# GJ0407790/cuda_ray_tracer

Measured on AMD Instinct MI355X. Metric: Mrays/sec, tenthousand.txt 1080p@16spp, higher is better.
Workload: dtype f32

## Files before the change

### cuda_ray_tracer_amd/api.py

```python
import contextlib
import ctypes as C
import os

from .binding import (LIB_PATH, EXPORTS, MIRT_ERR_ARG, MIRT_RENDER_COUNTERS, MIRT_HIT_NONE, MIRT_HIT_SPHERE, MIRT_HIT_TRIANGLE,
                      MIRT_HIT_PLANE, MIRT_QUERY_ANY_HIT, MIRT_DENOISE_SIGMA_C, MIRT_DENOISE_SIGMA_N, MIRT_DENOISE_SIGMA_P, MirtError, Vec3, Ray,
                      Hit, Camera, Shading, SceneDesc, RenderParams, Stats, MultiStats, TreeNode, lib, _check)

_F32, _U8, _INT, _HIT = ("float32",), ("uint8",), ("int32", "uint32"), ("float32", "int32", "uint32")


def _struct_with(cls, s, fields, what):
    out = cls.from_buffer_copy(bytes(s))
    names = dict(cls._fields_)
    for k, v in fields.items():
        if k not in names:
            raise ValueError(f"{k} is not a {what} field; expected one of {sorted(names)}")
        if names[k] is Vec3 and not isinstance(v, Vec3):
            v = Vec3(*(float(c) for c in v))
        setattr(out, k, v)
    return out


def _camera_with(cam, fields):
    return _struct_with(Camera, cam, fields, "camera")
# ... 79 lines not shown
        self._h = h
        self.build_ms = None

    def stats(self):
        st = Stats()
        _check(lib().mirt_get_stats(self._h, C.byref(st)))
        return st.as_dict()

    def set_option(self, name, value):
        _check(lib().mirt_scene_set_option(self._h, name.encode(), int(value)))

    def get_option(self, name):
        v = C.c_int(0)
        _check(lib().mirt_scene_get_option(self._h, name.encode(), C.byref(v)))
        return v.value

    def camera(self):
        cam = Camera()
        _check(lib().mirt_scene_get_camera(self._h, C.byref(cam)))
        return cam

    def set_camera(self, cam=None, **fields):
        new = _camera_with(cam if cam is not None else self.camera(), fields)
        _check(lib().mirt_scene_set_camera(self._h, C.byref(new)))
        return new

    def lights(self):
        import numpy as np
        from . import layouts
        suns = np.zeros(self.desc.num_suns, dtype=layouts.LIGHT)
# ... 608 lines not shown
```

### cuda_ray_tracer_amd/csrc/api.hip

```cpp
#include "scene_dev.h"
#include "host_scene.h"
#include "material_flags.h"

#include <cmath>
#include <cstdlib>
#include <cstring>
#include <memory>
#include <new>
#include <string>
#include <vector>

using namespace mirt;

namespace {

template <typename T>
int upload(DevBuf<T>& dst, const std::vector<T>& src)
{
  if (src.empty()) return MIRT_OK;
  const int rc = dst.alloc(src.size(), "upload");
  if (rc != MIRT_OK) return rc;
  MIRT_HIP(hipMemcpy(dst, src.data(), sizeof(T) * src.size(), hipMemcpyHostToDevice));
  return MIRT_OK;
}
// ... 48 lines not shown
  for (const OptionDesc& d : OPTIONS)
    if (strcmp(d.name, name) == 0) {
      if (value < d.lo || value > d.hi) { set_error(std::string("mirt_scene_set_option: value out of range for ") + name); return MIRT_ERR_ARG; }
      sc->opt.*(d.field) = value;
      return MIRT_OK;
    }
  set_error(std::string("mirt_scene_set_option: unknown option ") + name);
  return MIRT_ERR_ARG;
}

int mirt_scene_get_option(const MirtScene* sc, const char* name, int* value)
{
  if (!sc || !name || !value) { set_error("mirt_scene_get_option: null argument"); return MIRT_ERR_ARG; }
  for (const OptionDesc& d : OPTIONS)
    if (strcmp(d.name, name) == 0) { *value = sc->opt.*(d.field); return MIRT_OK; }
  set_error(std::string("mirt_scene_get_option: unknown option ") + name);
  return MIRT_ERR_ARG;
}

int mirt_scene_create(const MirtSceneDesc* d, int device, MirtScene** out)
{
  try {
    return scene_create(d, device, out);
  } catch (const std::bad_alloc&) {
    set_error("mirt_scene_create: out of host memory");
    return MIRT_ERR_ARG;
  }
}

}
// ... 78 lines not shown
    sc->wnode_base = wnode_bytes ? (uint32_t)((nodes_bytes + sph_bytes + tri_bytes + 64 + qnode_bytes + 127) / 128 * 128) : 0u;
    sc->nodes = reinterpret_cast<float4*>(sc->heap.get());
  }
  MIRT_TRY(upload(sc->spheres, spheres)); MIRT_TRY(upload(sc->tris, tris));
  MIRT_TRY(upload(sc->tri_verts, verts)); MIRT_TRY(upload(sc->mats, mats));
  MIRT_TRY(upload(sc->refs_in, refs)); MIRT_TRY(upload(sc->planes, planes)); MIRT_TRY(upload(sc->suns, suns)); MIRT_TRY(upload(sc->bulbs, bulbs));
  if (N > 0) {
    const size_t n = (size_t)N;
    MIRT_TRY(sc->codes.alloc(n, "codes")); MIRT_TRY(sc->order.alloc(n, "order"));
    MIRT_TRY(sc->parent.alloc(2 * n - 1, "parent")); MIRT_TRY(sc->boxes.alloc(6 * (2 * n - 1), "boxes"));
    if (N > 1) { MIRT_TRY(sc->child_l.alloc(n - 1, "child_l")); MIRT_TRY(sc->child_r.alloc(n - 1, "child_r")); MIRT_TRY(sc->range.alloc(n - 1, "range")); }
    MIRT_TRY(sc->unit_prim.alloc((size_t)sc->Ns + 3 * (size_t)sc->Nt, "unit_prim"));
    MIRT_TRY(sc->tris_before.alloc(n + 1, "tris_before"));
  }
  MIRT_TRY(sc->bounds_keys.alloc(6, "bounds_keys"));
  MIRT_TRY(sc->qparams.alloc(9, "qparams"));
  MIRT_TRY(sc->tri_boxes.alloc(2 * (size_t)sc->Nt, "tri_boxes"));
  for (RenderCtx& c : sc->ctx) {
    MIRT_TRY(c.counters.alloc(16, "counters"));
    MIRT_HIP(hipMemset(c.counters, 0, 16 * sizeof(unsigned long long)));
  }
  MIRT_TRY(sc->ev0.create()); MIRT_TRY(sc->ev1.create()); MIRT_TRY(sc->so_ev.create());
  for (RenderCtx& c : sc->ctx) {
    MIRT_TRY(c.ev0.create()); MIRT_TRY(c.ev1.create()); MIRT_TRY(c.ev2.create()); MIRT_TRY(c.ev3.create()); MIRT_TRY(c.order_ev.create());
  }
  *out = owner.release();
  return MIRT_OK;
}

}
// ... 315 lines not shown
```

### cuda_ray_tracer_amd/csrc/lbvh_build.hip

```cpp
#include "scene_dev.h"
#include "host_scene.h"

#include <cstdio>
#include <cstring>

namespace mirt {

int hip_fail(hipError_t e, const char* what, const char* file, int line)
{
  char buf[512];
  snprintf(buf, sizeof(buf), "HIP error in %s at line %d: %s (%s)", file, line, hipGetErrorString(e), what);
  set_error(buf);
  return MIRT_ERR_HIP;
}

namespace {

constexpr int BLOCK = 256;

struct Box { float xmin, xmax, ymin, ymax, zmin, zmax; };

MIRT_DEV Box prim_box(uint32_t type, uint32_t id, const float4* __restrict__ spheres, const float4* __restrict__ tri_verts)
{
  Box b;
// ... 406 lines not shown
                                                              uint32_t* __restrict__ unit_prim)
{
  const int j = blockIdx.x * BLOCK + threadIdx.x;
  if (j >= n) return;
  const MirtPrimRef r = refs[order[j]];
  const size_t unit = (size_t)j + 2 * (size_t)tris_before[j];
  if (r.type == 0) {
    prim_region[unit] = spheres[r.id];
    unit_prim[unit] = r.id;
  } else {
    prim_region[unit + 0] = tris[3 * (size_t)r.id + 0];
    prim_region[unit + 1] = tris[3 * (size_t)r.id + 1];
    prim_region[unit + 2] = tris[3 * (size_t)r.id + 2];
    unit_prim[unit + 0] = 0x80000000u | r.id; unit_prim[unit + 1] = 0x80000000u | r.id; unit_prim[unit + 2] = 0x80000000u | r.id;
  }
}

__global__ void __launch_bounds__(BLOCK) refit_pack_kernel(int n, const uint32_t* __restrict__ order, const MirtPrimRef* __restrict__ refs,
                                                           const float4* __restrict__ spheres, const float4* __restrict__ tri_verts,
                                                           const uint32_t* __restrict__ child_l, const uint32_t* __restrict__ child_r,
                                                           const int* __restrict__ parent, uint32_t* __restrict__ arrived,
                                                           float* boxes, float4* __restrict__ nodes, const uint32_t* __restrict__ tris_before,
                                                           const uint2* __restrict__ range, uint32_t prim_base16, float4* __restrict__ tri_boxes)
{
  const int j = blockIdx.x * BLOCK + threadIdx.x;
  if (j >= n) return;
  const uint32_t leaf_base = (uint32_t)(n - 1);
  uint32_t cur = leaf_base + (uint32_t)j;
  const MirtPrimRef r = refs[order[j]];
  const Box b = prim_box(r.type, r.id, spheres, tri_verts);
// ... 44 lines not shown
{
  const int sblocks = (int)((n + SORT_TILE - 1) / SORT_TILE);
  uint32_t *hist = ws, *totals = ws + 256 * (size_t)sblocks;
  hipLaunchKernelGGL(radix_pass_kernel<false>, dim3(sblocks), dim3(BLOCK), 0, stream, keys_in, (const uint32_t*)nullptr, keys_out, vals_out, hist, hist, totals, (int)n, 0, sblocks);
  hipLaunchKernelGGL(row_scan_kernel, dim3(256), dim3(BLOCK), 0, stream, hist, totals, sblocks);
  hipLaunchKernelGGL(radix_pass_kernel<true>, dim3(sblocks), dim3(BLOCK), 0, stream, keys_in, (const uint32_t*)nullptr, keys_out, vals_out, hist, hist, totals, (int)n, 0, sblocks);
  MIRT_HIP(hipGetLastError());
  return MIRT_OK;
}

int build_lbvh(MirtScene* sc, hipStream_t stream)
{
  const int n = sc->N;
  sc->built = false;
  sc->root_ref = REF_NONE;
  if (n == 0) { sc->built = true; sc->build_ms = 0.0f; return MIRT_OK; }

  const int sblocks = (n + SORT_TILE - 1) / SORT_TILE;
  const size_t wwords = 4 * (size_t)n + 256 * (size_t)sblocks + 256 + (size_t)(n > 1 ? n - 1 : 0);
  if (sc->build_ws.cap() < wwords) MIRT_TRY(sc->build_ws.alloc(wwords, "build_ws"));
  MIRT_HIP(hipEventRecord(sc->ev0, stream));
  const int nblk = (n + BLOCK - 1) / BLOCK;
  if (!sc->opt.bounds_as_shipped) {
    static const uint32_t init_keys[6] = {0xffffffffu, 0xffffffffu, 0xffffffffu, 0u, 0u, 0u};
    MIRT_HIP(hipMemcpyAsync(sc->bounds_keys, init_keys, sizeof(init_keys), hipMemcpyHostToDevice, stream));
    const int bgrid = nblk < 512 ? nblk : 512;
    hipLaunchKernelGGL(prim_bounds_kernel, dim3(bgrid), dim3(BLOCK), 0, stream, sc->refs_in, sc->spheres, sc->tri_verts, n, sc->bounds_keys);
  } else {
    static const uint32_t shipped_keys[6] = {0xff800000u, 0xff800000u, 0xff800000u, 0x007fffffu, 0x007fffffu, 0x007fffffu};
    MIRT_HIP(hipMemcpyAsync(sc->bounds_keys, shipped_keys, sizeof(shipped_keys), hipMemcpyHostToDevice, stream));
  }
// ... 7 lines not shown
    const int shift = pass * 8;
    hipLaunchKernelGGL(radix_pass_kernel<false>, dim3(sblocks), dim3(BLOCK), 0, stream, ki, vi, ko, vo, hist, hist, totals, n, shift, sblocks);
    hipLaunchKernelGGL(row_scan_kernel, dim3(256), dim3(BLOCK), 0, stream, hist, totals, sblocks);
    hipLaunchKernelGGL(radix_pass_kernel<true>, dim3(sblocks), dim3(BLOCK), 0, stream, ki, vi, ko, vo, hist, hist, totals, n, shift, sblocks);
    uint32_t* t = ki; ki = ko; ko = t; t = vi; vi = vo; vo = t;
  }
  MIRT_HIP(hipMemcpyAsync(sc->codes, ki, sizeof(uint32_t) * n, hipMemcpyDeviceToDevice, stream));
  MIRT_HIP(hipMemcpyAsync(sc->order, vi, sizeof(uint32_t) * n, hipMemcpyDeviceToDevice, stream));

  uint32_t* arrived = totals + 256;
  if (n > 1) {
    MIRT_HIP(hipMemsetAsync(arrived, 0, sizeof(uint32_t) * (n - 1), stream));
    MIRT_HIP(hipMemsetAsync(sc->parent, 0xff, sizeof(int) * (2 * (size_t)n - 1), stream));
    const int kblk = (n - 1 + BLOCK - 1) / BLOCK;
    hipLaunchKernelGGL(karras_kernel, dim3(kblk), dim3(BLOCK), 0, stream, sc->codes, n, sc->child_l, sc->child_r, sc->parent, sc->range);
  } else {
    MIRT_HIP(hipMemsetAsync(sc->parent, 0xff, sizeof(int), stream));
  }
  const int scan_blocks = (n + SCAN_TILE - 1) / SCAN_TILE;
  uint32_t* const block_sums = k1;
  hipLaunchKernelGGL(tri_scan_kernel<false>, dim3(scan_blocks), dim3(BLOCK), 0, stream, n, sc->order, sc->refs_in, block_sums, sc->tris_before);
  hipLaunchKernelGGL(scan_sums_kernel, dim3(1), dim3(BLOCK), 0, stream, block_sums, scan_blocks);
  hipLaunchKernelGGL(tri_scan_kernel<true>, dim3(scan_blocks), dim3(BLOCK), 0, stream, n, sc->order, sc->refs_in, block_sums, sc->tris_before);
  hipLaunchKernelGGL(scatter_prims_kernel, dim3(nblk), dim3(BLOCK), 0, stream, n, sc->order, sc->refs_in, sc->tris_before, sc->spheres, sc->tris,
                     reinterpret_cast<float4*>(sc->heap + sc->prim_base), sc->unit_prim);
  hipLaunchKernelGGL(refit_pack_kernel, dim3(nblk), dim3(BLOCK), 0, stream, n, sc->order, sc->refs_in, sc->spheres, sc->tri_verts,
                     sc->child_l, sc->child_r, sc->parent, arrived, sc->boxes, sc->nodes, sc->tris_before, sc->range, sc->prim_base / 16u, sc->tri_boxes);
  sc->root_ref_q = REF_NONE;
  if (sc->qnode_base && n > 1 && !sc->opt.bounds_as_shipped) {
    const int kblk = (n - 1 + BLOCK - 1) / BLOCK;
// ... 3 lines not shown
  }
  sc->root_ref_w = REF_NONE;
  if (sc->wnode_base && n > 1 && !sc->opt.bounds_as_shipped) {
    const int kblk = (n - 1 + BLOCK - 1) / BLOCK;
    hipLaunchKernelGGL(pack_wnodes_kernel, dim3(kblk), dim3(BLOCK), 0, stream, n, sc->bounds_keys, sc->child_l, sc->child_r, sc->boxes,
                       sc->order, sc->refs_in, sc->tris_before, sc->range, reinterpret_cast<uint4*>(sc->heap + sc->wnode_base),
                       sc->qparams, sc->wnode_base / 16u, sc->prim_base / 16u);
    sc->root_ref_w = sc->wnode_base / 16u;
  }
  MIRT_HIP(hipGetLastError());
  MIRT_HIP(hipEventRecord(sc->ev1, stream));
  MIRT_HIP(hipStreamSynchronize(stream));
  MIRT_HIP(hipEventElapsedTime(&sc->build_ms, sc->ev0, sc->ev1));
  sc->coord_max = 0.0f;
  sc->grid_ok = false;
  if (n > 1) {
    float rec[12];
    MIRT_HIP(hipMemcpy(rec, sc->nodes, sizeof(rec), hipMemcpyDeviceToHost));
    for (float v : rec) sc->coord_max = fmaxf(sc->coord_max, fabsf(v));
    sc->grid_ok = true;
    for (int k = 0; k < 3; ++k) {
      const float lo = fminf(rec[2 * k], rec[6 + 2 * k]), hi = fmaxf(rec[2 * k + 1], rec[6 + 2 * k + 1]);
      if (!(fmaxf(fabsf(lo), fabsf(hi)) <= 64.0f * (hi - lo))) sc->grid_ok = false;
    }
  }
  sc->root_ref = (n == 1) ? (REF_LEAF | (sc->Nt ? REF_TRI : 0u) | (sc->prim_base / 16u)) : 0u;
  sc->built = true;
  return MIRT_OK;
}

int get_tree(MirtScene* sc, MirtTreeNode* nodes, uint32_t* codes, MirtPrimRef* refs, float* bounds)
// ... 39 lines not shown
```

### cuda_ray_tracer_amd/csrc/render.hip

```cpp
#include "scene_dev.h"
#include "host_scene.h"
#include "shade_common.h"

#include <algorithm>
#include <climits>
#include <cmath>
#include <cstdio>
#include <cstdlib>
#include <cstring>

namespace mirt {
namespace {

constexpr int RBLOCK = 256;
constexpr int MAX_SPP = 4096;
constexpr int MAX_SLAB_ARGS = 4;
#ifndef MIRT_WAVES_PER_SIMD
#define MIRT_WAVES_PER_SIMD 4
#endif
MIRT_DEV bool triangle_leaf_reached(const RenderArgs* __restrict__ ap, uint32_t off16, const f3& o, const f3& d, float t, float tmin, f3& inv)
{
  const RenderArgs* aq = ap;
  asm volatile("" : "+s"(aq));
  const uint32_t id = aq->unit_prim[off16 - aq->prim_base16] & 0x7fffffffu;
  const float4 b0 = aq->tri_boxes[2 * (size_t)id], b1 = aq->tri_boxes[2 * (size_t)id + 1];
  inv = mk3(1.0f / d.x, 1.0f / d.y, 1.0f / d.z);
  const float tx1 = (b0.x - o.x) * inv.x, tx2 = (b0.y - o.x) * inv.x;
  const float ty1 = (b0.z - o.y) * inv.y, ty2 = (b0.w - o.y) * inv.y;
  const float tz1 = (b1.x - o.z) * inv.z, tz2 = (b1.y - o.z) * inv.z;
  const float te = fmaxf(fmaxf(fminf(tx1, tx2), fminf(ty1, ty2)), fminf(tz1, tz2));
  const float tx = fminf(fminf(fmaxf(tx1, tx2), fmaxf(ty1, ty2)), fmaxf(tz1, tz2));
  return te < tx && tx > tmin && te < t;
}

template <bool COUNT, int TABLES, bool QN, int SPECX = 0>
__global__ void __launch_bounds__(TRACE_BLOCK, MIRT_WAVES_PER_SIMD) trace_kernel(const RenderArgs* __restrict__ ap, const HotArgs h)
{
  constexpr int SPEC = SPECX;
  constexpr bool NOTRI = (SPEC & SPEC_NOTRI) != 0;
  constexpr bool WIDE = QN && !NOTRI;
#define MIRT_HELD (QN && !(SPEC & SPEC_NOBULB) && h.reach_check && S.batch_pending && !S.trav && S.li >= h.num_suns && S.li < h.num_suns + h.num_bulbs && \
                   S.refbest != REF_NONE)
  __shared__ __attribute__((aligned(16))) unsigned char lds_raw[STACK_LDS * TRACE_BLOCK * 4];
  __shared__ uint4 lds_rng[2][TRACE_BLOCK];
  __shared__ uint4 lds_park[2][TRACE_BLOCK];
  uint32_t* const lds_stack = reinterpret_cast<uint32_t*>(lds_raw);
  const int tid = threadIdx.x;
  const int lane = tid & 63;
  (void)lane;
  const unsigned char* const heap = reinterpret_cast<const unsigned char*>(h.nodes);
  const uint32_t gid32 = blockIdx.x * (uint32_t)TRACE_BLOCK + (uint32_t)tid;
  const long long gid = (long long)gid32;
  const long long gthreads = (long long)(gridDim.x * (uint32_t)TRACE_BLOCK);
  Counters cn = {0, 0, 0, 0, 0, 0, 0, 0, 0};

// ... 10 lines not shown
  S.pc = 0; S.refr_bounce = 0; S.gi_n = 0; S.state = ST_PRIMARY;
  S.bo = mk3(0, 0, 0); S.rdir = mk3(0, 0, 1); S.li = 0; S.occl = 0ull; S.batch_pending = false; S.has_reflect = false;
  S.o = mk3(0, 0, 0); S.d = mk3(0, 0, 1); S.inv = mk3(0, 0, 1); S.bounce = 0; S.limit = INFINITY; S.shadow = false;
  S.tplane = INFINITY; S.plane_id = -1;
  S.qb = mk3(0, 0, 0); S.qc = mk3(0, 0, 0); S.qsx = S.qsy = S.qsz = 0;
  S.cur = REF_NONE; S.tos = REF_NONE; S.sp = 0; S.tbest = INFINITY; S.refbest = REF_NONE;

  lds_rng[0][tid] = make_uint4(0, 0, 0, 0);
  lds_rng[1][tid] = make_uint4(0, 0, 0, 0);
  lds_park[0][tid] = make_uint4(0, 0, 0, 0);
  lds_park[1][tid] = make_uint4(0, 0, 0, __float_as_uint(1.458f));
  for (;;) {
    const RenderArgs* aq = ap;
    asm volatile("" : "+s"(aq));
    const RenderArgs& a = *aq;
    if (a.reach_check && !S.trav && S.g >= 0 && !(exhausted && S.batch_pending && !MIRT_HELD) && (!S.batch_pending || S.li >= a.num_suns)) {
      if (hit_needs_literal_walk<QN>(a, S)) walk_literally<COUNT, NOTRI>(a, S, cn, gid, gthreads);
    }
    {
      const uint4 r0 = lds_rng[0][tid], r1 = lds_rng[1][tid];
      S.rng.v0 = r0.x; S.rng.v1 = r0.y; S.rng.v2 = r0.z; S.rng.v3 = r0.w;
      S.rng.v4 = r1.x; S.rng.d = r1.y; S.rng.bm_extra = __uint_as_float(r1.z); S.rng.bm_flag = (int)r1.w;
      const uint4 p0 = lds_park[0][tid], p1 = lds_park[1][tid];
      S.L = mk3(__uint_as_float(p0.x), __uint_as_float(p0.y), __uint_as_float(p0.z)); S.alpha = __uint_as_float(p0.w);
      S.wD = mk3(__uint_as_float(p1.x), __uint_as_float(p1.y), __uint_as_float(p1.z)); S.Hior = __uint_as_float(p1.w);
    }
    for (;;) {
      const bool live = !S.trav && S.g >= 0 && !(exhausted && S.batch_pending && !MIRT_HELD);
      if (__ballot(live) == 0) break;
      if (live && S.batch_pending) batch_next<COUNT, QN, RenderArgs, SPEC>(a, S, cn);
// ... 45 lines not shown
      if (exhausted && __ballot(S.g >= 0) == 0) break;
      continue;
    }

    const float tmin = 0.0001f;
    for (;;) {
      const unsigned long long tm = __ballot(S.trav);
      const bool pend = !S.trav && S.batch_pending && !MIRT_HELD;
      const unsigned long long bm = __ballot(pend);
      if (tm == 0 && bm == 0) break;
      const int nwait = __popcll(__ballot(!S.trav && !pend && (S.g >= 0 || !exhausted)));
      const int nlive = __popcll(__ballot(S.g >= 0));
      const bool drain = exhausted && nlive <= h.drain_lanes;
      if (nwait >= h.refill_k || (drain && nwait > 0)) break;
      if (bm != 0 && (__popcll(bm) >= h.batch_k || tm == 0 || drain)) {
        if (pend) batch_next<COUNT, QN, HotArgs, SPEC>(h, S, cn);
      }
      const bool leaf0 = S.trav && (S.cur & REF_LEAF) != 0;
      const unsigned long long lm = __ballot(leaf0);
      const bool do_leaf0 = __popcll(lm) >= h.leaf_k || __ballot(S.trav && !leaf0) == 0 || drain;
      for (int rep = 0; rep < h.reps; ++rep) {
      const bool leaf = S.trav && (S.cur & REF_LEAF) != 0;
      const bool do_leaf = rep == 0 && do_leaf0;
      if (S.trav && (!leaf || do_leaf)) {
        if (COUNT) ++S.steps;
        const float4* rec = reinterpret_cast<const float4*>(heap + (S.cur << 4));
        bool pop = false;
        if (leaf) {
          float t = 0.0f;
          bool hit = false;
          const float4 q0 = rec[0];
          const bool tri = !NOTRI && (S.cur & REF_TRI) != 0;
          if (tri) {
            if (COUNT) cn.tri_tests++;
            const float4 q1 = rec[1], q2 = rec[2];
            hit = triangle_hit(q0, q1, q2, S.o, S.d, t);
// ... 13 lines not shown
              S.tbest = INFINITY; S.refbest = REF_NONE;
            }
          }
          S.tbest = closer ? t : S.tbest;
          S.refbest = closer ? S.cur : S.refbest;
          S.trav = !(closer && S.shadow && t < S.limit);
          pop = S.trav;
        } else {
          if (COUNT) cn.internal_visits++;
          uint32_t noff = S.cur << 4;
          asm volatile("" : "+v"(noff));
          const float4* nrec = reinterpret_cast<const float4*>(heap + noff);
          bool hl, hr;
          float tel, ter;
          uint32_t lref, rref;
#define MIRT_PUSH(v) do { if (S.sp < h.lds_depth) lds_stack[S.sp * TRACE_BLOCK + tid] = S.tos; \
                          else h.stack_spill[(size_t)(S.sp - h.lds_depth) * gthreads + gid] = S.tos; \
                          S.tos = (v); ++S.sp; if (COUNT) cn.max_stack = max(cn.max_stack, (uint32_t)S.sp); } while (0)
          if (WIDE && S.qsx != 0u) {
            const uint4 w0 = *reinterpret_cast<const uint4*>(nrec), w1 = *reinterpret_cast<const uint4*>(nrec + 1);
            const uint4 w2 = *reinterpret_cast<const uint4*>(nrec + 2), w3 = *reinterpret_cast<const uint4*>(nrec + 3);
            const bool h0 = box_q(w0.x, w0.y, w0.z, S.inv, S.qb, S.qc, S.qsx, S.qsy, S.qsz, S.tbest, tmin);
            const bool h1 = box_q(w0.w, w1.x, w1.y, S.inv, S.qb, S.qc, S.qsx, S.qsy, S.qsz, S.tbest, tmin);
            const bool h2 = box_q(w1.z, w1.w, w2.x, S.inv, S.qb, S.qc, S.qsx, S.qsy, S.qsz, S.tbest, tmin);
            const bool h3 = box_q(w2.y, w2.z, w2.w, S.inv, S.qb, S.qc, S.qsx, S.qsy, S.qsz, S.tbest, tmin);
            uint32_t cand = w3.w;
            bool have = h3;
            if (h2 && have) MIRT_PUSH(cand);
            cand = h2 ? w3.z : cand; have = have || h2;
            if (h1 && have) MIRT_PUSH(cand);
            cand = h1 ? w3.y : cand; have = have || h1;
// ... 7 lines not shown
            order_children(hl, hr, tel, ter, NODE_SWAP_ANY | NODE_SWAP_PURE, h.swap_mask, lref, rref);
          } else {
            const float4 q0 = nrec[0], q1 = nrec[1], q2 = nrec[2];
            const uint4 ch = *reinterpret_cast<const uint4*>(nrec + 3);
            box_pair(q0, q1, q2, S.o.x, S.o.y, S.o.z, S.inv.x, S.inv.y, S.inv.z, S.tbest, tmin, hl, hr, tel, ter);
            lref = ch.x; rref = ch.y;
            if (!QN) order_children(hl, hr, tel, ter, ch.z, h.swap_mask, lref, rref);
          }
          const bool both = hl && hr;
          if (both) MIRT_PUSH(rref);
#undef MIRT_PUSH
          S.cur = hl ? lref : (hr ? rref : S.cur);
          pop = !(hl || hr);
        }
        if (pop) {
          S.trav = S.sp != 0;
          S.cur = S.tos;
          S.sp = S.sp > 0 ? S.sp - 1 : 0;
          S.tos = lds_stack[(S.sp < h.lds_depth ? S.sp : 0) * TRACE_BLOCK + tid];
          if (S.sp >= h.lds_depth) S.tos = h.stack_spill[(size_t)(S.sp - h.lds_depth) * gthreads + gid];
        }
      }
      }
    }
  }

  unsigned long long* const counters = COUNT ? ap->counters : nullptr;
  if (COUNT && counters) {
    uint32_t v[9] = {cn.samples, cn.rays, cn.shadow_rays, cn.internal_visits, cn.sphere_tests, cn.tri_tests, cn.mat_fetches, cn.max_stack, cn.traversed};
#pragma unroll
    for (int k = 0; k < 9; ++k) {
      unsigned long long x = v[k];
      if (k == 7) {
#pragma unroll
        for (int off = 32; off > 0; off >>= 1) { unsigned long long y = __shfl_xor(x, off); x = x > y ? x : y; }
// ... 206 lines not shown

struct RenderCall {
  MirtScene* sc; const MirtRenderParams* p;
  void* d_rgba8; void* d_rgba_f32; void* d_accum; const AdaptiveArgs* ax;
  int sample_first, sample_count;
  hipStream_t stream;
  bool sparse() const { return ax && ax->list; }
  bool count() const { return (p->flags & MIRT_RENDER_COUNTERS) != 0; }
};

static int scene_facts(MirtScene* sc, SceneFacts* out)
{
  const int rc = settle_facts(sc);
  if (rc != MIRT_OK) return rc;
  SceneFacts f;
  f.N = sc->N; f.Nt = sc->Nt; f.grid_ok = sc->grid_ok;
  f.has_quantised = sc->root_ref_q != REF_NONE; f.has_wide = sc->root_ref_w != REF_NONE;
  f.colors_finite = sc->colors_finite; f.any_trans = sc->any_trans; f.any_rough = sc->any_rough;
  f.gi = sc->d.gi; f.bounces = sc->d.bounces; f.num_suns = sc->d.num_suns; f.num_bulbs = sc->d.num_bulbs;
  *out = f;
  return MIRT_OK;
}

static int check_call(const RenderCall& c, int64_t* npix)
{
  const char* who = c.ax ? "mirt_render_accumulate_pixels" : (c.d_accum ? "mirt_render_accumulate" : "mirt_render");
  *npix = 0;
  if (!c.sc->built) { set_error(std::string(who) + ": call mirt_build_lbvh first"); return MIRT_ERR_STATE; }
  const int64_t n = local_pixels(c.p);
  if (n < 0 || c.p->spp < 0 || (!c.d_rgba8 && !c.d_accum)) { set_error(std::string(who) + ": bad parameters"); return MIRT_ERR_ARG; }
  if (c.sample_first < 0 || c.sample_count < 1 || (long long)c.sample_first + c.sample_count > MAX_SPP) {
// ... 165 lines not shown

static int sample_table_finish(MirtScene* sc, hipStream_t stream)
{
  MIRT_HIP(hipEventRecord(sc->so_ev, stream));
  sc->so_key = sc->so_pending_key; sc->so_busy = true;
  return MIRT_OK;
}

using TraceKernel = void (*)(const RenderArgs*, HotArgs);
template <bool C, bool Q, int P>
static TraceKernel trace_kernel_tables(bool t8) { return t8 ? trace_kernel<C, 8, Q, P> : trace_kernel<C, 4, Q, P>; }
template <bool C>
static TraceKernel trace_kernel_spec(bool t8, const CallPlan& pl)
{
  const bool both = pl.nobulb && pl.nopend;
  if (pl.qn && pl.notri) return both ? trace_kernel_tables<C, true, SPEC_NOTRI | SPEC_NOBULB | SPEC_NOPEND>(t8) : trace_kernel_tables<C, true, SPEC_NOTRI>(t8);
  if (pl.qn) return both ? trace_kernel_tables<C, true, SPEC_NOBULB | SPEC_NOPEND>(t8) : pl.nobulb ? trace_kernel_tables<C, true, SPEC_NOBULB>(t8) : trace_kernel_tables<C, true, 0>(t8);
  return both ? trace_kernel_tables<C, false, SPEC_NOBULB | SPEC_NOPEND>(t8) : pl.nobulb ? trace_kernel_tables<C, false, SPEC_NOBULB>(t8) : trace_kernel_tables<C, false, 0>(t8);
}
static TraceKernel trace_kernel_for(bool count, bool t8, const CallPlan& pl) { return count ? trace_kernel_spec<true>(t8, pl) : trace_kernel_spec<false>(t8, pl); }

static int launch_slab(const RenderCall& c, RenderCtx& cx, const CallPlan& pl, RenderArgs& a, const HotArgs& h, int slab, long long p0, long long pn,
                       int blocks, TraceKernel kernel)
{
  const hipStream_t stream = c.stream;
  if (c.sc->opt.wavefront != 0) {
    float tms = 0.0f;
    int rc = wavefront_trace(c.sc, cx, a, c.count(), stream, &tms);
    if (rc != MIRT_OK) return rc;
    cx.wf_trace_ms = (cx.wf_trace_ms < 0.0f ? 0.0f : cx.wf_trace_ms) + tms;
// ... 78 lines not shown
    if (measure_chunks) a.chunk_cost = cx.chunk_cost;
  } else if (pl.hand_out == HAND_BY_SAMPLE) {
    rc = sample_table_find(sc, pl, okey, &ordered_samples, &measure_samples);
  }
  if (rc != MIRT_OK) return rc;
  const TraceKernel kernel = trace_kernel_for(count || measure_chunks || measure_samples,
                                              a.needs_rng && a.rng.mode == 0 && a.rng.chunk_bits == 8, pl);

  cx.frame_id = ++sc->frame_seq;
  MIRT_HIP(hipEventRecord(cx.ev0, stream));
  if (measure_chunks) MIRT_HIP(hipMemsetAsync(cx.chunk_cost, 0, 4 * nchunks, stream));
  if (count) { MIRT_HIP(hipMemsetAsync(cx.counters, 0, 8 * sizeof(unsigned long long), stream)); MIRT_HIP(hipMemsetAsync(cx.counters + 11, 0, sizeof(unsigned long long), stream)); }
  cx.wf_trace_ms = -1.0f;
  cx.launches = pl.nslabs;
  cx.node_bytes = pl.node_bytes;
  MIRT_HIP(hipEventRecord(cx.ev1, stream));
  for (int slab = 0; slab < pl.nslabs; ++slab) {
    const long long p0 = (long long)slab * pl.slab_pixels;
    const long long pn = (p0 + pl.slab_pixels < npix ? p0 + pl.slab_pixels : npix) - p0;
    a.pixel_base = p0; a.num_local_pixels = pn; a.num_samples = pn * sample_count;
    a.sample_order = ordered_samples ? sc->so_order + (size_t)p0 * sample_count : nullptr;
    a.sample_key = measure_samples ? sc->so_keys : nullptr;
    if (c.sparse()) {
      a.sample_order = cx.sp_table;
      a.num_samples = (pn < pl.listed_max ? pn : pl.listed_max) * sample_count;
    }
    rc = launch_slab(c, cx, pl, a, h, slab, p0, pn, blocks, kernel);
    if (rc != MIRT_OK) return rc;
    if (slab == pl.nslabs - 1) MIRT_HIP(hipEventRecord(cx.ev2, stream));
    rc = resolve_slab(c, cx, p0, pn);
// ... 99 lines not shown
```

### cuda_ray_tracer_amd/csrc/render_plan.h

```cpp
#ifndef MIRT_RENDER_PLAN_H
#define MIRT_RENDER_PLAN_H

#include <cstdint>

#ifndef MIRT_TRACE_BLOCK
#define MIRT_TRACE_BLOCK 64
#endif
#ifndef MIRT_STACK_LDS
#define MIRT_STACK_LDS 24
#endif

namespace mirt {

constexpr int TRACE_BLOCK = MIRT_TRACE_BLOCK;
constexpr int STACK_LDS = MIRT_STACK_LDS;
constexpr int MAX_CHUNK_SHIFT = 8, MIN_CHUNK_SHIFT = 6;
constexpr uint32_t NODE_SWAP_PURE = 1u;
constexpr uint32_t NODE_SWAP_ANY = 2u;

struct Options {
  int bounds_as_shipped = 0;
  int traversal = 1;
  int wavefront = 0;
  int stack_lds_depth = -1;
  int refill_k = 0;
  int batch_k = 8, drain_lanes = 16;
  int leaf_k = 0;
  int reps = 0;
  int init_k = 0;
  int chunk_shift = 0;
// ... 2 lines not shown
  int skip_unlit = 1;
  int qnodes = 1;
  int specialise = 1;
  int sched = 2;
  int slab_log2 = 28;
  int wf_pool = 1 << 21, wf_refill_k = 16;
};

struct SceneFacts {
  int N = 0, Nt = 0;
  bool grid_ok = false;
  bool has_quantised = false, has_wide = false;
  bool colors_finite = true, any_trans = false, any_rough = false;
  int gi = 0, bounces = 0;
  int num_suns = 0, num_bulbs = 0;
};

struct CallShape {
  long long npix = 0;
  int sample_first = 0, sample_count = 1;
  int spp = 0;
  bool accumulate = false;
  long long num_listed = -1;
  bool counters = false;
};

enum HandOut {
  HAND_FRAME = 0,
  HAND_LIST,
  HAND_BY_CHUNK,
// ... 6 lines not shown
  long long listed_max = 0;
  long long launch_samples_max = 0;
  long long total_samples = 0;
  bool per_pixel_seed = false;
  int args_spp = 0;
  int rng_sample_tables = 0;
  bool shading_rng = false;
  bool notri = false, qn = false;
  uint32_t swap_mask = 0;
  int reach_check = 0;
  int node_bytes = 64;
  bool nobulb = false, nopend = false;
  bool need_pending = false; int pending_slots = 0;
  int skip_unlit = 0, shadow_anyhit = 0;
  int refill_k = 0, init_k = 0, leaf_k = 0, reps = 0, lds_depth = 0;
  HandOut hand_out = HAND_FRAME;
};

inline CallPlan plan_call(const SceneFacts& s, const Options& opt, const CallShape& c)
{
  CallPlan pl;
  const bool sparse = c.num_listed >= 0;
  const bool wavefront = opt.wavefront != 0;
  pl.slab_pixels = (1ll << opt.slab_log2) / c.sample_count;
  if (pl.slab_pixels < 1) pl.slab_pixels = 1;
  if (pl.slab_pixels > c.npix) pl.slab_pixels = c.npix;
  pl.nslabs = (int)((c.npix + pl.slab_pixels - 1) / pl.slab_pixels);
  pl.slab_samples_max = pl.slab_pixels * c.sample_count;
  pl.listed_max = sparse ? (c.num_listed < pl.slab_pixels ? c.num_listed : pl.slab_pixels) : 0;
  pl.launch_samples_max = sparse ? pl.listed_max * c.sample_count : pl.slab_samples_max;
// ... 8 lines not shown
  pl.qn = s.grid_ok && (pl.notri ? (qwant && opt.traversal >= 1 && s.has_quantised)
                                 : (qwant && opt.traversal == 1 && s.has_wide && (opt.qnodes >= 2 || s.N >= 65536)));
  pl.swap_mask = opt.traversal == 1 ? ((pl.qn && pl.notri) ? NODE_SWAP_PURE : 0u) : (opt.traversal == 2 ? NODE_SWAP_ANY : 0u);
  pl.reach_check = (pl.qn && s.N > 1) ? 1 : 0;
  pl.node_bytes = (pl.qn && pl.notri) ? 32 : 64;

  pl.need_pending = s.any_trans || s.gi != 0;
  pl.pending_slots = pl.need_pending ? 2 * (s.bounces + (s.gi > 0 ? s.gi : 0) + 2) : 0;
  const bool specialise = opt.specialise != 0 && s.colors_finite;
  pl.nobulb = specialise && s.num_bulbs == 0;
  pl.nopend = specialise && !pl.need_pending;
  pl.skip_unlit = (opt.skip_unlit != 0 && s.colors_finite && s.num_suns + s.num_bulbs <= 32) ? 1 : 0;
  pl.shadow_anyhit = opt.shadow_anyhit != 0 ? 1 : 0;

  pl.lds_depth = (opt.stack_lds_depth >= 0 && opt.stack_lds_depth <= STACK_LDS) ? opt.stack_lds_depth : STACK_LDS;
  pl.refill_k = opt.refill_k > 0 ? opt.refill_k : (pl.qn ? (pl.notri ? 32 : 24) : 64);
  const int init_k = opt.init_k > 0 ? opt.init_k : (pl.qn ? (pl.notri ? 10 : 8) : 64);
  pl.init_k = init_k < pl.refill_k ? init_k : pl.refill_k;
  pl.leaf_k = opt.leaf_k > 0 ? opt.leaf_k : (pl.qn ? 8 : 4);
  pl.reps = opt.reps > 0 ? opt.reps : ((pl.qn && !pl.notri) ? 5 : 4);

  if (sparse) pl.hand_out = HAND_LIST;
  else if (wavefront) pl.hand_out = HAND_FRAME;
  else if (opt.sched == 1 && pl.nslabs == 1) pl.hand_out = HAND_BY_CHUNK;
  else if (opt.sched == 2 && pl.slab_samples_max < 0x7fffffffll && pl.total_samples <= (3ll << 30)) pl.hand_out = HAND_BY_SAMPLE;
  return pl;
}

inline int plan_chunk_shift(long long launch_samples_max, int blocks, int option)
{
// ... 8 lines not shown
```

### cuda_ray_tracer_amd/csrc/scene_dev.h

```cpp
#ifndef MIRT_SCENE_DEV_H
#define MIRT_SCENE_DEV_H

#include <hip/hip_runtime.h>
#include <string>
#include <vector>

#include "../../include/mirt.h"
#include "dev_mem.h"
#include "device_common.h"
#include "render_plan.h"
#include "xorwow_tables.h"

namespace mirt {

constexpr uint32_t REF_LEAF = 0x80000000u;
constexpr uint32_t REF_TRI = 0x40000000u;
constexpr uint32_t REF_OFFMASK = 0x0fffffffu;
constexpr uint32_t REF_NONE = 0xf0000000u;
constexpr float QGRID = 65535.0f;
constexpr uint32_t REF_QPURE = 0x20000000u;
constexpr uint32_t QBOX_NONE = 0x0000ffffu;
constexpr int STACK_TOTAL_WIDE = 88;
constexpr float QINV_STEPS = 1152921504606846976.0f;

// ... 143 lines not shown
  mirt::DevBuf<float> boxes;
  float4* nodes = nullptr;
  mirt::DevBuf<unsigned char> heap;
  uint32_t prim_base = 0;
  mirt::DevBuf<uint32_t> unit_prim;
  mirt::DevBuf<uint32_t> tris_before;
  mirt::DevBuf<uint2> range;
  uint32_t qnode_base = 0;
  uint32_t wnode_base = 0;
  uint32_t root_ref_w = mirt::REF_NONE;
  uint32_t root_ref_q = mirt::REF_NONE;
  mirt::DevBuf<float> qparams;
  mirt::DevBuf<float4> tri_boxes;
  mirt::DevBuf<uint32_t> build_ws;
  mirt::DevBuf<uint32_t> bounds_keys;
  uint32_t root_ref = mirt::REF_NONE;
  bool built = false;
  float build_ms = 0.0f;
  float coord_max = 0.0f;
  bool grid_ok = false;
  mirt::RenderCtx ctx[mirt::MIRT_MAX_FRAMES];
  unsigned frame_no = 0;
  unsigned long long frame_seq = 0;
  mirt::RenderCtx* last = nullptr;
  unsigned long long overflow_events = 0;
  double trace_ms_sum = 0.0; int trace_frames = 0;
  mirt::DevBuf<uint32_t> wf_state;
  mirt::DevBuf<float4> wf_rays;
  mirt::DevBuf<unsigned long long> wf_ctr;
  mirt::PinnedBuf<unsigned long long> wf_ctr_host;
  std::vector<mirt::Event> wf_events;
  int wf_rounds = 0;
  mirt::DevBuf<uint32_t> so_order, so_keys, so_keys2, so_ws;
  long long so_key = -1, so_pending_key = -1, so_total = -1; mirt::Event so_ev; bool so_busy = false;
  mirt::RngCache rng;
// ... 104 lines not shown
```

Before: 8934.

## Specialise trace kernel to an LDS-only stack when BVH depth fits

Computes the binary BVH's maximum leaf depth on the GPU at build time and stores it on the scene. When the depth fits in the LDS stack and the walk is not wide, the render plan picks a kernel variant that drops the global spill path, uses a sentinel top-of-stack in place of the sp==0 check, and rebuilds some hot args from the constant block to relieve register pressure. It adds a depth kernel plus a sync readback to the build, and more template instantiations. It relies on the depth bound to guarantee the stack never overflows LDS.

```diff
diff --git a/cuda_ray_tracer_amd/api.py b/cuda_ray_tracer_amd/api.py
--- a/cuda_ray_tracer_amd/api.py
+++ b/cuda_ray_tracer_amd/api.py
@@ -117,6 +117,10 @@
         v = C.c_int(0)
         _check(lib().mirt_scene_get_option(self._h, name.encode(), C.byref(v)))
         return v.value
+
+    def stack_info(self):
+        return {"tree_depth": self.get_option("tree_depth"), "lds_capacity": self.get_option("stack_lds_capacity"),
+                "lds_only": bool(self.get_option("stack_lds_only"))}
 
     def camera(self):
         cam = Camera()
diff --git a/cuda_ray_tracer_amd/csrc/api.hip b/cuda_ray_tracer_amd/csrc/api.hip
--- a/cuda_ray_tracer_amd/csrc/api.hip
+++ b/cuda_ray_tracer_amd/csrc/api.hip
@@ -86,6 +86,9 @@
   if (!sc || !name || !value) { set_error("mirt_scene_get_option: null argument"); return MIRT_ERR_ARG; }
   for (const OptionDesc& d : OPTIONS)
     if (strcmp(d.name, name) == 0) { *value = sc->opt.*(d.field); return MIRT_OK; }
+  if (strcmp(name, "tree_depth") == 0) { *value = sc->built ? sc->tree_depth : -1; return MIRT_OK; }
+  if (strcmp(name, "stack_lds_capacity") == 0) { *value = STACK_LDS_CAPACITY; return MIRT_OK; }
+  if (strcmp(name, "stack_lds_only") == 0) { *value = sc->last_lds_only ? 1 : 0; return MIRT_OK; }
   set_error(std::string("mirt_scene_get_option: unknown option ") + name);
   return MIRT_ERR_ARG;
 }
@@ -194,6 +197,7 @@
     MIRT_TRY(sc->tris_before.alloc(n + 1, "tris_before"));
   }
   MIRT_TRY(sc->bounds_keys.alloc(6, "bounds_keys"));
+  MIRT_TRY(sc->depth_dev.alloc(1, "depth_dev"));
   MIRT_TRY(sc->qparams.alloc(9, "qparams"));
   MIRT_TRY(sc->tri_boxes.alloc(2 * (size_t)sc->Nt, "tri_boxes"));
   for (RenderCtx& c : sc->ctx) {
diff --git a/cuda_ray_tracer_amd/csrc/lbvh_build.hip b/cuda_ray_tracer_amd/csrc/lbvh_build.hip
--- a/cuda_ray_tracer_amd/csrc/lbvh_build.hip
+++ b/cuda_ray_tracer_amd/csrc/lbvh_build.hip
@@ -444,6 +444,19 @@
     prim_region[unit + 2] = tris[3 * (size_t)r.id + 2];
     unit_prim[unit + 0] = 0x80000000u | r.id; unit_prim[unit + 1] = 0x80000000u | r.id; unit_prim[unit + 2] = 0x80000000u | r.id;
   }
+}
+
+__global__ void __launch_bounds__(BLOCK) tree_depth_kernel(int n, const int* __restrict__ parent, uint32_t* __restrict__ depth)
+{
+  const int j = blockIdx.x * BLOCK + threadIdx.x;
+  uint32_t d = 0;
+  if (j < n) {
+    int p = parent[n - 1 + j];
+    while (p >= 0 && p < n - 1 && d < 255u) { ++d; p = parent[p]; }
+  }
+#pragma unroll
+  for (int off = 32; off > 0; off >>= 1) d = max(d, (uint32_t)__shfl_xor((int)d, off));
+  if ((threadIdx.x & 63) == 0 && d > 0) atomicMax(depth, d);
 }
 
 __global__ void __launch_bounds__(BLOCK) refit_pack_kernel(int n, const uint32_t* __restrict__ order, const MirtPrimRef* __restrict__ refs,
@@ -518,7 +531,8 @@
   const int n = sc->N;
   sc->built = false;
   sc->root_ref = REF_NONE;
-  if (n == 0) { sc->built = true; sc->build_ms = 0.0f; return MIRT_OK; }
+  sc->tree_depth = -1;
+  if (n == 0) { sc->built = true; sc->build_ms = 0.0f; sc->tree_depth = 0; return MIRT_OK; }
 
   const int sblocks = (n + SORT_TILE - 1) / SORT_TILE;
   const size_t wwords = 4 * (size_t)n + 256 * (size_t)sblocks + 256 + (size_t)(n > 1 ? n - 1 : 0);
@@ -556,6 +570,8 @@
     MIRT_HIP(hipMemsetAsync(sc->parent, 0xff, sizeof(int) * (2 * (size_t)n - 1), stream));
     const int kblk = (n - 1 + BLOCK - 1) / BLOCK;
     hipLaunchKernelGGL(karras_kernel, dim3(kblk), dim3(BLOCK), 0, stream, sc->codes, n, sc->child_l, sc->child_r, sc->parent, sc->range);
+    MIRT_HIP(hipMemsetAsync(sc->depth_dev, 0, sizeof(uint32_t), stream));
+    hipLaunchKernelGGL(tree_depth_kernel, dim3(nblk), dim3(BLOCK), 0, stream, n, sc->parent, sc->depth_dev);
   } else {
     MIRT_HIP(hipMemsetAsync(sc->parent, 0xff, sizeof(int), stream));
   }
@@ -589,7 +605,11 @@
   MIRT_HIP(hipEventElapsedTime(&sc->build_ms, sc->ev0, sc->ev1));
   sc->coord_max = 0.0f;
   sc->grid_ok = false;
+  sc->tree_depth = 0;
   if (n > 1) {
+    uint32_t depth = 0;
+    MIRT_HIP(hipMemcpy(&depth, sc->depth_dev, sizeof(depth), hipMemcpyDeviceToHost));
+    sc->tree_depth = (int)depth;
     float rec[12];
     MIRT_HIP(hipMemcpy(rec, sc->nodes, sizeof(rec), hipMemcpyDeviceToHost));
     for (float v : rec) sc->coord_max = fmaxf(sc->coord_max, fabsf(v));
diff --git a/cuda_ray_tracer_amd/csrc/render.hip b/cuda_ray_tracer_amd/csrc/render.hip
--- a/cuda_ray_tracer_amd/csrc/render.hip
+++ b/cuda_ray_tracer_amd/csrc/render.hip
@@ -33,12 +33,15 @@
   return te < tx && tx > tmin && te < t;
 }
 
+constexpr int SPEC_LDS_STACK = 8;
 template <bool COUNT, int TABLES, bool QN, int SPECX = 0>
 __global__ void __launch_bounds__(TRACE_BLOCK, MIRT_WAVES_PER_SIMD) trace_kernel(const RenderArgs* __restrict__ ap, const HotArgs h)
 {
-  constexpr int SPEC = SPECX;
+  constexpr int SPEC = SPECX & ~SPEC_LDS_STACK;
+  constexpr bool LDS_ONLY = (SPECX & SPEC_LDS_STACK) != 0;
   constexpr bool NOTRI = (SPEC & SPEC_NOTRI) != 0;
   constexpr bool WIDE = QN && !NOTRI;
+  static_assert(!(LDS_ONLY && WIDE), "the wide walk pushes up to three entries per step: the depth of the tree does not bound its stack");
 #define MIRT_HELD (QN && !(SPEC & SPEC_NOBULB) && h.reach_check && S.batch_pending && !S.trav && S.li >= h.num_suns && S.li < h.num_suns + h.num_bulbs && \
                    S.refbest != REF_NONE)
   __shared__ __attribute__((aligned(16))) unsigned char lds_raw[STACK_LDS * TRACE_BLOCK * 4];
@@ -79,6 +82,7 @@
     const RenderArgs* aq = ap;
     asm volatile("" : "+s"(aq));
     const RenderArgs& a = *aq;
+    if (LDS_ONLY && !S.trav) S.tos = REF_NONE;
     if (a.reach_check && !S.trav && S.g >= 0 && !(exhausted && S.batch_pending && !MIRT_HELD) && (!S.batch_pending || S.li >= a.num_suns)) {
       if (hit_needs_literal_walk<QN>(a, S)) walk_literally<COUNT, NOTRI>(a, S, cn, gid, gthreads);
     }
@@ -154,12 +158,26 @@
       const bool drain = exhausted && nlive <= h.drain_lanes;
       if (nwait >= h.refill_k || (drain && nwait > 0)) break;
       if (bm != 0 && (__popcll(bm) >= h.batch_k || tm == 0 || drain)) {
-        if (pend) batch_next<COUNT, QN, HotArgs, SPEC>(h, S, cn);
+        if (LDS_ONLY) {
+          if (pend) {
+            const RenderArgs* hq = ap;
+            asm volatile("" : "+s"(hq));
+            HotArgs hh = h;
+            hh.suns = hq->suns; hh.root_ref = hq->root_ref; hh.num_planes = hq->num_planes; hh.num_suns = hq->num_suns; hh.num_bulbs = hq->num_bulbs;
+            hh.shadow_anyhit = hq->shadow_anyhit;
+            batch_next<COUNT, QN, HotArgs, SPEC>(hh, S, cn);
+            S.tos = REF_NONE;
+          }
+        } else {
+          if (pend) batch_next<COUNT, QN, HotArgs, SPEC>(h, S, cn);
+        }
       }
       const bool leaf0 = S.trav && (S.cur & REF_LEAF) != 0;
       const unsigned long long lm = __ballot(leaf0);
       const bool do_leaf0 = __popcll(lm) >= h.leaf_k || __ballot(S.trav && !leaf0) == 0 || drain;
-      for (int rep = 0; rep < h.reps; ++rep) {
+      int reps = h.reps;
+      if (LDS_ONLY) asm volatile("" : "+s"(reps));
+      for (int rep = 0; rep < reps; ++rep) {
       const bool leaf = S.trav && (S.cur & REF_LEAF) != 0;
       const bool do_leaf = rep == 0 && do_leaf0;
       if (S.trav && (!leaf || do_leaf)) {
@@ -203,7 +221,7 @@
           bool hl, hr;
           float tel, ter;
           uint32_t lref, rref;
-#define MIRT_PUSH(v) do { if (S.sp < h.lds_depth) lds_stack[S.sp * TRACE_BLOCK + tid] = S.tos; \
+#define MIRT_PUSH(v) do { if (LDS_ONLY || S.sp < h.lds_depth) lds_stack[S.sp * TRACE_BLOCK + tid] = S.tos; \
                           else h.stack_spill[(size_t)(S.sp - h.lds_depth) * gthreads + gid] = S.tos; \
                           S.tos = (v); ++S.sp; if (COUNT) cn.max_stack = max(cn.max_stack, (uint32_t)S.sp); } while (0)
           if (WIDE && S.qsx != 0u) {
@@ -241,11 +259,18 @@
           pop = !(hl || hr);
         }
         if (pop) {
-          S.trav = S.sp != 0;
-          S.cur = S.tos;
-          S.sp = S.sp > 0 ? S.sp - 1 : 0;
-          S.tos = lds_stack[(S.sp < h.lds_depth ? S.sp : 0) * TRACE_BLOCK + tid];
-          if (S.sp >= h.lds_depth) S.tos = h.stack_spill[(size_t)(S.sp - h.lds_depth) * gthreads + gid];
+          if (LDS_ONLY) {
+            S.cur = S.tos;
+            S.trav = S.cur != REF_NONE;
+            S.sp = (int)__builtin_elementwise_sub_sat((uint32_t)S.sp, 1u);
+            S.tos = lds_stack[S.sp * TRACE_BLOCK + tid];
+          } else {
+            S.trav = S.sp != 0;
+            S.cur = S.tos;
+            S.sp = S.sp > 0 ? S.sp - 1 : 0;
+            S.tos = lds_stack[(S.sp < h.lds_depth ? S.sp : 0) * TRACE_BLOCK + tid];
+            if (S.sp >= h.lds_depth) S.tos = h.stack_spill[(size_t)(S.sp - h.lds_depth) * gthreads + gid];
+          }
         }
       }
       }
@@ -482,7 +507,7 @@
   const int rc = settle_facts(sc);
   if (rc != MIRT_OK) return rc;
   SceneFacts f;
-  f.N = sc->N; f.Nt = sc->Nt; f.grid_ok = sc->grid_ok;
+  f.N = sc->N; f.Nt = sc->Nt; f.grid_ok = sc->grid_ok; f.tree_depth = sc->tree_depth;
   f.has_quantised = sc->root_ref_q != REF_NONE; f.has_wide = sc->root_ref_w != REF_NONE;
   f.colors_finite = sc->colors_finite; f.any_trans = sc->any_trans; f.any_rough = sc->any_rough;
   f.gi = sc->d.gi; f.bounces = sc->d.bounces; f.num_suns = sc->d.num_suns; f.num_bulbs = sc->d.num_bulbs;
@@ -678,6 +703,11 @@
 static TraceKernel trace_kernel_spec(bool t8, const CallPlan& pl)
 {
   const bool both = pl.nobulb && pl.nopend;
+  if (pl.lds_only) {
+    constexpr int L = SPEC_LDS_STACK;
+    if (pl.qn) return both ? trace_kernel_tables<C, true, L | SPEC_NOTRI | SPEC_NOBULB | SPEC_NOPEND>(t8) : trace_kernel_tables<C, true, L | SPEC_NOTRI>(t8);
+    return both ? trace_kernel_tables<C, false, L | SPEC_NOBULB | SPEC_NOPEND>(t8) : pl.nobulb ? trace_kernel_tables<C, false, L | SPEC_NOBULB>(t8) : trace_kernel_tables<C, false, L>(t8);
+  }
   if (pl.qn && pl.notri) return both ? trace_kernel_tables<C, true, SPEC_NOTRI | SPEC_NOBULB | SPEC_NOPEND>(t8) : trace_kernel_tables<C, true, SPEC_NOTRI>(t8);
   if (pl.qn) return both ? trace_kernel_tables<C, true, SPEC_NOBULB | SPEC_NOPEND>(t8) : pl.nobulb ? trace_kernel_tables<C, true, SPEC_NOBULB>(t8) : trace_kernel_tables<C, true, 0>(t8);
   return both ? trace_kernel_tables<C, false, SPEC_NOBULB | SPEC_NOPEND>(t8) : pl.nobulb ? trace_kernel_tables<C, false, SPEC_NOBULB>(t8) : trace_kernel_tables<C, false, 0>(t8);
@@ -786,6 +816,7 @@
   cx.wf_trace_ms = -1.0f;
   cx.launches = pl.nslabs;
   cx.node_bytes = pl.node_bytes;
+  sc->last_lds_only = pl.lds_only;
   MIRT_HIP(hipEventRecord(cx.ev1, stream));
   for (int slab = 0; slab < pl.nslabs; ++slab) {
     const long long p0 = (long long)slab * pl.slab_pixels;
diff --git a/cuda_ray_tracer_amd/csrc/render_plan.h b/cuda_ray_tracer_amd/csrc/render_plan.h
--- a/cuda_ray_tracer_amd/csrc/render_plan.h
+++ b/cuda_ray_tracer_amd/csrc/render_plan.h
@@ -14,6 +14,7 @@
 
 constexpr int TRACE_BLOCK = MIRT_TRACE_BLOCK;
 constexpr int STACK_LDS = MIRT_STACK_LDS;
+constexpr int STACK_LDS_CAPACITY = STACK_LDS;
 constexpr int MAX_CHUNK_SHIFT = 8, MIN_CHUNK_SHIFT = 6;
 constexpr uint32_t NODE_SWAP_PURE = 1u;
 constexpr uint32_t NODE_SWAP_ANY = 2u;
@@ -46,6 +47,7 @@
   bool colors_finite = true, any_trans = false, any_rough = false;
   int gi = 0, bounces = 0;
   int num_suns = 0, num_bulbs = 0;
+  int tree_depth = -1;
 };
 
 struct CallShape {
@@ -82,6 +84,7 @@
   bool need_pending = false; int pending_slots = 0;
   int skip_unlit = 0, shadow_anyhit = 0;
   int refill_k = 0, init_k = 0, leaf_k = 0, reps = 0, lds_depth = 0;
+  bool lds_only = false;
   HandOut hand_out = HAND_FRAME;
 };
 
@@ -120,6 +123,7 @@
   pl.shadow_anyhit = opt.shadow_anyhit != 0 ? 1 : 0;
 
   pl.lds_depth = (opt.stack_lds_depth >= 0 && opt.stack_lds_depth <= STACK_LDS) ? opt.stack_lds_depth : STACK_LDS;
+  pl.lds_only = !wavefront && opt.stack_lds_depth < 0 && (!pl.qn || pl.notri) && s.tree_depth >= 0 && s.tree_depth <= STACK_LDS_CAPACITY;
   pl.refill_k = opt.refill_k > 0 ? opt.refill_k : (pl.qn ? (pl.notri ? 32 : 24) : 64);
   const int init_k = opt.init_k > 0 ? opt.init_k : (pl.qn ? (pl.notri ? 10 : 8) : 64);
   pl.init_k = init_k < pl.refill_k ? init_k : pl.refill_k;
diff --git a/cuda_ray_tracer_amd/csrc/scene_dev.h b/cuda_ray_tracer_amd/csrc/scene_dev.h
--- a/cuda_ray_tracer_amd/csrc/scene_dev.h
+++ b/cuda_ray_tracer_amd/csrc/scene_dev.h
@@ -181,11 +181,14 @@
   mirt::DevBuf<float4> tri_boxes;
   mirt::DevBuf<uint32_t> build_ws;
   mirt::DevBuf<uint32_t> bounds_keys;
+  mirt::DevBuf<uint32_t> depth_dev;
   uint32_t root_ref = mirt::REF_NONE;
   bool built = false;
   float build_ms = 0.0f;
   float coord_max = 0.0f;
   bool grid_ok = false;
+  int tree_depth = -1;
+  bool last_lds_only = false;
   mirt::RenderCtx ctx[mirt::MIRT_MAX_FRAMES];
   unsigned frame_no = 0;
   unsigned long long frame_seq = 0;
```

After: 9264 (median of 6 runs). 1.04x the previous value.
